# jianwang-mpi/GlobalEgoMocap

Hardware: AMD Instinct MI355X
Metric: optimised windows/sec (10-frame, 15-joint) (higher is better)
Workload: dtype f32

## Files before the change

globalegomocap_amd/csrc/decoder_bf16.hip:

```cpp
#include "gem_internal.h"
#include "gemm_glds.h"
#include "gemm_big.h"

namespace gem {

using glds::Args;
namespace bf16a = glds;

__global__ void f32_to_bf16_kernel(const float* __restrict__ src, uint16_t* __restrict__ dst, size_t n4) {
    const size_t i = (size_t)blockIdx.x * blockDim.x + threadIdx.x;
    if (i >= n4) return;
    const bf16a::f32x4 v = reinterpret_cast<const bf16a::f32x4*>(src)[i];
    reinterpret_cast<bf16a::u32x2*>(dst)[i] = bf16a::u32x2{bf16a::pack_bf16(v[0], v[1]), bf16a::pack_bf16(v[2], v[3])};
}
int launch_f32_to_bf16(const float* src, uint16_t* dst, size_t n, hipStream_t s) {
    const size_t n4 = n / 4;
    if (!n4) return 0;
    hipLaunchKernelGGL(f32_to_bf16_kernel, dim3((unsigned)((n4 + 255) / 256)), dim3(256), 0, s, src, dst, n4);
    GEM_HIP(hipGetLastError());
    return 0;
}

__global__ void f32_split_bf16_kernel(const float* __restrict__ src, uint16_t* __restrict__ hi, uint16_t* __restrict__ lo, size_t n) {
    const size_t i = (size_t)blockIdx.x * blockDim.x + threadIdx.x;
// ... 251 lines not shown
                               nullptr, true, false)) return 1;
                in = w.dec_act_b[i];
            }
        }
        TailArgs ta;
        plan_tail(net.dec, st, T, h->J, &ta);
        ta.B = B; ta.forward_only = forward_only ? 1 : 0; ta.dbg_ts = nullptr;
        ta.in_slab = in_slab; ta.in_bias = front ? net.front.bias : net.dec[st - 1].bias;
        ta.in_bias_ld = front ? net.dec[0].N : 0;
        for (int i = 0; i < ta.n; ++i) {
            const Layer& f = net.dec[st + i];
            const Layer& g = net.dec_bwd[st + i];
            ta.fwd[i] = TailLayerDev{f.w4, f.bias, f.K, f.N};
            ta.bwd[i] = TailLayerDev{g.w4, nullptr, g.K, g.N};
        }
        ta.a_in = w.dec_act[st - 1]; ta.g_out = nullptr; ta.g_out_b = w.dec_grad_b[st];
        ta.Xp = (w.dyn && !forward_only) ? nullptr : w.dec_act.back();
        ta.e = ea;
        if (launch_tail(h, ta, net.tail_lds, s)) return 1;
        if (forward_only) return 0;
        back_from = st - 1;
        gin = w.dec_grad_b[st];
    } else {
        if (front) {
            if (gemm_bf16a(h, net.front, EPI_BIAS_LRELU, w.trial_b, h->Dp, nullptr, w.dec_act_b[0], true, net.front.N, B, s, 0, perm, true, false))
                return 1;
            in = w.dec_act_b[0];
        }
        for (int i = front ? 1 : 0; i < n_dec; ++i) {
            const bool last = i + 1 == n_dec;
// ... 30 lines not shown
```

globalegomocap_amd/csrc/gem_api.hip:

```cpp
#include <cxxabi.h>

#include <algorithm>
#include <cmath>
#include <cstdio>
#include <cstdlib>
#include <cstring>
#include <memory>

#include "gem_internal.h"

namespace gem {

static thread_local std::string g_error;
void set_error(const std::string& msg) { g_error = msg; }
bool hip_ok(hipError_t e, const char* what) {
    if (e == hipSuccess) return true;
    g_error = std::string(what) + ": " + hipGetErrorString(e);
    return false;
}

const char* dev_env(const char* name) {
    const char* on = getenv("GEM_DEV");
    if (!on || on[0] != '1') return nullptr;
    return getenv(name);
// ... 398 lines not shown
        net.dec_bwd.push_back(Lb);
        return 0;
    };
    for (int i = nh - 1; i >= 1; --i)
        if (add_dec(c.hidden[i], c.hidden[i - 1], true, true)) return 1;
    if (add_dec(c.hidden[0], c.hidden[0], true, true)) return 1;
    if (add_dec(c.hidden[0], C, false, false)) return 1;
    net.tail_start = -1;
    if (!dev_env("GEM_NO_TAIL"))
        for (int st = 1; st < (int)net.dec.size(); ++st) {
            const size_t bytes = plan_tail(net.dec, st, T, h->J, nullptr);
            if (bytes && bytes <= 160 * 1024) { net.tail_start = st; net.tail_lds = bytes; break; }
        }
    if (net.tail_start == 1 && !dev_env("GEM_NO_FRONT") && compose_front(h, net, first_conv, dec_in_bias_tm.data())) return 1;
    if (build_tail_bf16_stream(h, net)) return 1;
    net.host_fwd.clear(); net.host_fwd.shrink_to_fit();
    net.host_bwd.clear(); net.host_bwd.shrink_to_fit();
    net.loaded = true;
    return 0;
}

}

namespace gem {

static int check_call(gem_handle* h, int stage, int B, const char* who) {
    if (!h) { set_error(std::string(who) + ": null handle"); return 1; }
    if (stage < 0 || stage > 1 || !h->net[stage].loaded) { set_error(std::string(who) + ": VAE weights of this stage are not loaded"); return 1; }
    if (B < 0 || B > h->ws.Bmax) { set_error(std::string(who) + ": B exceeds max_windows"); return 1; }
    GEM_HIP(hipSetDevice(h->cfg.device));
// ... 109 lines not shown
            if (rc) return 1;
            in = w.dec_act[i];
        }
    }
    TailArgs ta;
    const size_t tail_lds = plan_tail_for(h, net.dec, st, tail_wgs, &ta);
    ta.B = B; ta.forward_only = forward_only ? 1 : 0; ta.dbg_ts = nullptr;
    ta.in_slab = in_slab; ta.in_bias = front ? net.front.bias : net.dec[st - 1].bias;
    ta.in_bias_ld = front ? net.dec[0].N : 0;
    for (int i = 0; i < ta.n; ++i) {
        const Layer& f = net.dec[st + i];
        const Layer& g = net.dec_bwd[st + i];
        ta.fwd[i] = TailLayerDev{f.w4, f.bias, f.K, f.N};
        ta.bwd[i] = TailLayerDev{g.w4, nullptr, g.K, g.N};
    }
    ta.a_in = w.dec_act[st - 1]; ta.g_out = w.dec_grad[st]; ta.g_out_b = nullptr; ta.Xp = (w.dyn && !forward_only) ? nullptr : w.dec_act.back();
    ta.e = ea;
    if (launch_tail(h, ta, tail_lds, s)) return 1;
    if (forward_only) return 0;
    if (front) {
        w.defer_reduce = w.dyn;
        const int rc = launch_gemm(h, net.front_bwd, EPI_BIAS, w.dec_grad[st], net.front_bwd.K, nullptr, w.dz, h->Dp, B, h->T, s, 0);
        w.grad_slab = w.defer_reduce ? w.deferred : SlabSrc{};
        w.defer_reduce = false;
        return rc;
    }
    return decoder_backward(h, stage, B, s, st - 1, w.dec_grad[st]);
}

struct StageRun {
// ... 483 lines not shown
```

globalegomocap_amd/csrc/gem_internal.h:

```cpp
#pragma once
#if defined(__HIP_DEVICE_COMPILE__) && !defined(GEM_NO_PACKED_FP32)
#error "compile with: -Xclang -target-feature -Xclang -packed-fp32-ops -DGEM_NO_PACKED_FP32 (__graft_entry__.NO_PACKED_FP32)"
#endif

#include <hip/hip_runtime.h>
#include <stdint.h>
#include <atomic>
#include <set>
#include <string>
#include <vector>

#include "../../include/gem_hip.h"

namespace gem {

constexpr int PAD = 64;
constexpr float LEAKY_SLOPE = 0.01f;
constexpr double BN_EPS = 1e-5;
constexpr int MAX_HIST = 128;
constexpr int MAXJ_ERR = GEM_MAX_JOINTS;
constexpr int N_LOG = 1 << 16;
constexpr int TRACE_ROUNDS = 64;

inline int pad64(int x) { return (x + PAD - 1) / PAD * PAD; }
// ... 17 lines not shown

struct StageNet {
    bool loaded = false;
    std::vector<Layer> enc;
    Layer fc;
    Layer dec_in;
    std::vector<Layer> dec;
    Layer dec_in_bwd;
    std::vector<Layer> dec_bwd;
    Layer front, front_bwd;
    int tail_start = -1;
    size_t tail_lds = 0;
    uint16_t* tb_stream = nullptr;
    int tb_steps_f = 0, tb_steps_b = 0;
    size_t tb_lds = 0;
    std::vector<std::vector<float>> host_fwd, host_bwd;
    std::vector<void*> allocs;
};

struct alignas(16) LbfgsState {
    int phase, n_iter, evals, ls_iter, ls_evals, max_ls, first_bracket, ls_done, insuf, low, high;
    int hist_count, hist_start, nan_seen;
    double loss, prev_loss, t, gtd, d_norm, H_diag;
    double t_prev, f_prev, gtd_prev;
    double br_t[2], br_f[2], br_gtd[2];
    double ro[MAX_HIST];
    double cadj[MAX_HIST];
};

struct SlabSrc {
// ... 220 lines not shown
struct TailLayerDev { const float* w4; const float* bias; int K, N; };
struct TailArgs {
    int n, B, G, forward_only, escr, mask_first;
    int waves, rows;
    SlabSrc in_slab;
    const float* in_bias;
    int in_bias_ld;
    long long* dbg_ts;
    TailLayerDev fwd[TAIL_MAX_LAYERS], bwd[TAIL_MAX_LAYERS];
    const float* a_in;
    float* g_out;
    uint16_t* g_out_b;
    float* Xp;
    int off_act[TAIL_MAX_LAYERS + 1], ld_act[TAIL_MAX_LAYERS + 1], off_g[2], ld_g, off_red, off_escr, off_zero, off_pre;
    EnergyArgs e;
};
size_t plan_tail(const std::vector<Layer>& dec, int start, int T, int J, TailArgs* out, bool shared = false);
size_t plan_tail_for(const gem_handle* h, const std::vector<Layer>& dec, int start, int wgs, TailArgs* out);

constexpr int TB_MAX_LAYERS = 6;
struct TailB16Layer { int K, N; const float* bias; };
struct TailB16Args {
    int n, B, G, nrt, forward_only, mask_first;
    SlabSrc in_slab;
    const float* in_bias;
    int in_bias_ld;
    const uint16_t* a_in_b;
    uint16_t* g_out_b;
    float* Xp;
    long long* dbg_ts;
    const uint16_t* wstream;
    int steps_f, steps_total;
    TailB16Layer fwd[TB_MAX_LAYERS], bwd[TB_MAX_LAYERS];
    int off_act[TB_MAX_LAYERS + 1], ld_act[TB_MAX_LAYERS + 1];
    int off_mask[TB_MAX_LAYERS], ld_mask[TB_MAX_LAYERS];
    int off_x, escr, off_mb, off_zero, off_tab;
    int off_bwin, off_epair;
    EnergyArgs e;
};
size_t plan_tail_bf16(const std::vector<Layer>& dec, int start, int T, int J, TailB16Args* out, int nrt = 5);
int tail_bf16_row_tiles(const gem_handle* h, int B, int T);
int build_tail_bf16_stream(gem_handle* h, StageNet& net);
int launch_tail_bf16(gem_handle* h, const TailB16Args& a, size_t lds_bytes, hipStream_t s);
int launch_tail(gem_handle* h, const TailArgs& a, size_t lds_bytes, hipStream_t s);
int tail_cap_workgroups(const gem_handle* h, const std::vector<Layer>& dec, int start);
int launch_mean_bone(gem_handle* h, const float* pose, int n_frames, float* out, hipStream_t s);
int launch_gather_windows(const float* frames, const int32_t* frame0, float* out, int B, int T, int JC, hipStream_t s);
int launch_relative_global(const float* local, const double* cams, const int32_t* frame0, float* rel, int B, int T, int J,
                           hipStream_t s);
int launch_to_global(const float* rel, const double* cams, const int32_t* frame0, double* out, int B, int T, int J,
                     hipStream_t s);

int launch_errors(gem_handle* h, const double* est, const double* mid, const double* opt, const double* gt, int F,
                  const double* bone_mm, double* frame_out, double* out, hipStream_t s, int n_seq);
int launch_merge(const double* win, double* tmp, double* out, int n_chunks, int wpc, int T, int JC, int overlap, int smooth,
                 hipStream_t s);
size_t errors_frame_lds_bytes(int J);
// ... 12 lines not shown
```

globalegomocap_amd/csrc/tail.hip:

```cpp
#include <algorithm>

#include "energy_device.h"

namespace gem {

typedef float f32x16 __attribute__((ext_vector_type(16)));
typedef float f32x4 __attribute__((ext_vector_type(4)));

__device__ __forceinline__ float bf16_round(float x) {
    const __bf16 b = (__bf16)x;
    return (float)b;
}

constexpr int TAIL_WAVES = 8;
constexpr int TAIL_THREADS = TAIL_WAVES * 64;
constexpr int TAIL_WAVES_SHARED = 4;

constexpr int TAIL_ROWS = 16;

template <int W>
__device__ __forceinline__ void tail_prefetch_first(const TailLayerDev L, f32x4 (&dst)[4]) {
    const int lane = threadIdx.x & 63, wave = __builtin_amdgcn_readfirstlane(threadIdx.x >> 6);
    const int c = lane & 15, q = lane >> 4;
    const int n0 = wave * 16;
// ... 95 lines not shown
__device__ __forceinline__ void tail_gemm(const float* in, int ld_in, const float* zero_line, const TailLayerDev L,
                                          const TailLayerDev next, bool has_next, int T, int R, f32x4 (&bpre)[4], Epi epi) {
    if constexpr (W == TAIL_WAVES_SHARED) {
        if (L.N > 32 * W) {
            tail_gemm_nt<W, 2>(in, ld_in, zero_line, L, next, false, T, R, bpre, epi);
            tail_gemm_nt<W, 2>(in, ld_in, zero_line, L, next, has_next, T, R, bpre, epi, 32 * W, false);
        } else if (L.N > 16 * W) tail_gemm_nt<W, 2>(in, ld_in, zero_line, L, next, has_next, T, R, bpre, epi);
        else tail_gemm_nt<W, 1>(in, ld_in, zero_line, L, next, has_next, T, R, bpre, epi);
    } else {
        if (L.N > 32 * W) tail_gemm_nt<W, 4>(in, ld_in, zero_line, L, next, has_next, T, R, bpre, epi);
        else if (L.N > 16 * W) tail_gemm_nt<W, 2>(in, ld_in, zero_line, L, next, has_next, T, R, bpre, epi);
        else tail_gemm_nt<W, 1>(in, ld_in, zero_line, L, next, has_next, T, R, bpre, epi);
    }
}

template <int NL, int W>
__global__ __launch_bounds__(64 * W, W == TAIL_WAVES_SHARED ? 3 : 2) void decoder_tail_kernel(TailArgs a) {
    constexpr int THREADS = 64 * W;
    constexpr bool TIGHT = W == TAIL_WAVES_SHARED;
    constexpr int STAGE_U = 2048 / THREADS;
    constexpr int PRE_E = TAIL_THREADS / THREADS;
    extern __shared__ __attribute__((aligned(16))) float lds[];
    const int tid = threadIdx.x, lane = tid & 63, wave = __builtin_amdgcn_readfirstlane(tid >> 6);
    const int T = a.e.T;
    int probe = 0;
#define TAIL_PROBE()                                                                                   \
    if (a.dbg_ts && blockIdx.x == 0 && tid == 0) {                                                     \
        a.dbg_ts[2 * probe] = clock64();                                                               \
        a.dbg_ts[2 * probe + 1] = wall_clock64();                                                      \
        ++probe;                                                                                       \
    }
    const int w0 = blockIdx.x * a.G;
    const int B = a.e.n_dev ? *a.e.n_dev : a.B;
    if (w0 >= B) return;
    const int nwin = min(a.G, B - w0);
    const int R = nwin * T;
    const size_t row0 = (size_t)w0 * T;

    {
        const int K0 = a.fwd[0].K, q4 = K0 / 4, n4 = (TIGHT ? a.rows : TAIL_ROWS) * q4;
        float* dst = lds + a.off_act[0];
        if (a.in_slab.base) {
            int nslab;
            size_t stride;
            slab_layout(a.in_slab, nslab, stride);
            for (int u = 0; u < STAGE_U; ++u) {
                const int i = tid + u * THREADS, r = i / q4, c = (i - r * q4) * 4;
                if (i >= n4) break;
                f32x4 v = {0.f, 0.f, 0.f, 0.f};
                if (r < R) {
                    const float* p = a.in_slab.base + (row0 + r) * K0 + c;
                    for (int z0 = 0; z0 < nslab; z0 += 8) {
                        f32x4 t[8];
#pragma unroll
                        for (int k = 0; k < 8; ++k) t[k] = *reinterpret_cast<const f32x4*>(p + (size_t)min(z0 + k, nslab - 1) * stride);
// ... 10 lines not shown
        } else {
            f32x4 v[STAGE_U];
#pragma unroll
            for (int u = 0; u < STAGE_U; ++u) {
                const int i = tid + u * THREADS, r = i / q4, c = (i - r * q4) * 4;
                v[u] = f32x4{0.f, 0.f, 0.f, 0.f};
                if (i < n4 && r < R) v[u] = *reinterpret_cast<const f32x4*>(a.a_in + (row0 + r) * K0 + c);
            }
#pragma unroll
            for (int u = 0; u < STAGE_U; ++u) {
                const int i = tid + u * THREADS, r = i / q4, c = (i - r * q4) * 4;
                if (i < n4) *reinterpret_cast<f32x4*>(dst + r * a.ld_act[0] + c) = v[u];
            }
        }
        if (tid < 64) lds[a.off_zero + tid] = 0.f;
    }
    float pre_x0[PRE_E], pre_mb = 0.f;
    int pre_par = 0, pre_ch[PRE_E];
#pragma unroll
    for (int k = 0; k < PRE_E; ++k) { pre_x0[k] = 0.f; pre_ch[k] = -1; }
    static_assert(MAXJ * MAXJ <= TAIL_THREADS && MAXJ <= 64, "the children table is parked by PRE_E passes of the workgroup");
    const bool pre_on = a.G == 1 && !a.forward_only && T * a.e.J * 3 <= TAIL_THREADS;
    if (pre_on) {
        const int J = a.e.J, n = T * J * 3, bw = a.e.perm ? a.e.perm[w0] : w0;
#pragma unroll
        for (int k = 0; k < PRE_E; ++k) {
            const int e = tid + k * THREADS;
            if (e < n) pre_x0[k] = a.e.X0[(size_t)bw * n + e];
            if (e < J * MAXJ) pre_ch[k] = a.e.children[e];
        }
        if (tid < J) { pre_mb = a.e.mean_bone[(size_t)bw * J + tid]; pre_par = a.e.parents[tid]; }
    }
    TAIL_PROBE();
    __syncthreads();
    TAIL_PROBE();

    f32x4 bpre[4];
    tail_prefetch_first<W>(a.fwd[0], bpre);
#pragma unroll
    for (int i = 0; i < NL; ++i) {
        const bool last = (i + 1 == NL);
        float* out = lds + a.off_act[i + 1];
        const int ldo = a.ld_act[i + 1];
        float* Xp = last ? a.Xp : nullptr;
        const TailLayerDev nxt = !last ? a.fwd[i + 1 < NL ? i + 1 : i] : a.bwd[NL - 1];
        tail_gemm<W>(lds + a.off_act[i], a.ld_act[i], lds + a.off_zero, a.fwd[i], nxt, !last || !a.forward_only, T, R, bpre,
                  [&](const f32x4& acc, int r0, int col, float bv) {
#pragma unroll
                      for (int e = 0; e < 4; ++e) {
                          float v = acc[e] + bv;
                          if (!last) v = v > 0.f ? v : v * LEAKY_SLOPE;
                          if (!TIGHT || r0 + e < a.rows) out[(r0 + e) * ldo + col] = v;
                          if (Xp && r0 + e < R) Xp[(row0 + r0 + e) * PAD + col] = v;
                      }
                  });
        if (i == 0 && pre_on) {
            const int J = a.e.J, n = T * J * 3;
            float* pre = lds + a.off_pre;
            int* prei = reinterpret_cast<int*>(pre + n + J);
#pragma unroll
            for (int k = 0; k < PRE_E; ++k) {
                const int e = tid + k * THREADS;
                if (e < n) pre[e] = pre_x0[k];
                if (e < J * MAXJ) prei[J + e] = pre_ch[k];
            }
            if (tid < J) { pre[n + tid] = pre_mb; prei[tid] = pre_par; }
        }
        __syncthreads();
        TAIL_PROBE();
    }
    if (a.forward_only) return;

    float* g_cur = lds + a.off_g[0];
    float* g_nxt = lds + a.off_g[1];
    if (a.G == 1) {
        float* scr = lds + a.off_escr;
        const int J = a.e.J, n = T * J * 3;
        const float* pre = lds + a.off_pre;
        const int* prei = reinterpret_cast<const int*>(pre + n + J);
        if (T == 10 && J == 15)
            energy_window<true, THREADS, 10, 15>(a.e, a.e.perm ? a.e.perm[w0] : w0, tid, lds + a.off_act[NL], a.ld_act[NL], scr,
                                                      scr + a.escr, scr + 2 * a.escr, scr + 3 * a.escr, g_cur, a.ld_g, a.fwd[NL - 1].N,
                                                      nullptr, pre_on ? pre : nullptr, pre_on ? pre + n : nullptr, pre_on ? prei : nullptr,
                                                      pre_on ? prei + J : nullptr);
        else
            energy_window<true, THREADS>(a.e, a.e.perm ? a.e.perm[w0] : w0, tid, lds + a.off_act[NL], a.ld_act[NL], scr,
                                              scr + a.escr, scr + 2 * a.escr, scr + 3 * a.escr, g_cur, a.ld_g, a.fwd[NL - 1].N,
                                              nullptr, pre_on ? pre : nullptr, pre_on ? pre + n : nullptr, pre_on ? prei : nullptr,
                                              pre_on ? prei + J : nullptr);
    } else if (wave < nwin) {
        float* scr = lds + a.off_escr + wave * 4 * a.escr;
        energy_window<false>(a.e, a.e.perm ? a.e.perm[w0 + wave] : w0 + wave, lane,
                             lds + a.off_act[NL] + wave * T * a.ld_act[NL], a.ld_act[NL], scr, scr + a.escr,
                             scr + 2 * a.escr, scr + 3 * a.escr, g_cur + wave * T * a.ld_g, a.ld_g, a.fwd[NL - 1].N);
    }
    __syncthreads();
    TAIL_PROBE();

#pragma unroll
    for (int i = NL - 1; i >= 0; --i) {
        const float* act = lds + a.off_act[i];
        const int lda = a.ld_act[i];
        const int ldg = a.ld_g;
        float* gout = a.g_out;
        uint16_t* gout_b = a.g_out_b;
        const int K0 = a.fwd[0].K;
        tail_gemm<W>(g_cur, a.ld_g, lds + a.off_zero, a.bwd[i], a.bwd[i > 0 ? i - 1 : 0], i > 0, T, R, bpre,
                  [&](const f32x4& acc, int r0, int col, float) {
#pragma unroll
                      for (int e = 0; e < 4; ++e) {
                          const int row = r0 + e;
                          const float v = (i > 0 || a.mask_first) ? acc[e] * (act[row * lda + col] > 0.f ? 1.f : LEAKY_SLOPE) : acc[e];
                          if (i > 0) { if (!TIGHT || row < a.rows) g_nxt[row * ldg + col] = v; }
                          else if (row < R) {
                              if (gout_b) gout_b[(row0 + row) * K0 + col] = (uint16_t)(__builtin_bit_cast(unsigned int, bf16_round(v)) >> 16);
                              else gout[(row0 + row) * K0 + col] = v;
                          }
                      }
                  });
        __syncthreads();
        TAIL_PROBE();
        float* t = g_cur; g_cur = g_nxt; g_nxt = t;
    }
#undef TAIL_PROBE
}

size_t plan_tail(const std::vector<Layer>& dec, int start, int T, int J, TailArgs* out, bool shared) {
    const int n = (int)dec.size() - start;
    if (start < 0 || n < 1 || n > TAIL_MAX_LAYERS || T > TAIL_ROWS) return 0;
    for (int i = start; i < (int)dec.size(); ++i) {
        const int K = dec[i].K, N = dec[i].N;
        auto ok = [](int v) { return v == 64 || v == 128 || v == 256 || v == 512; };
        if (!ok(K) || !ok(N)) return 0;
    }
    TailArgs a{};
    a.n = n;
    a.mask_first = start > 0;
    a.G = TAIL_ROWS / T;
    if (shared && a.G != 1) return 0;
// ... 7 lines not shown
        a.ld_act[i] = width + 4;
        off += rows * (width + 4);
        if (i >= 1 && width > maxg) maxg = width;
    }
    a.ld_g = maxg + 4;
    a.off_g[0] = off; off += rows * a.ld_g;
    a.off_g[1] = off; off += rows * a.ld_g;
    a.escr = (T * J * 3 + 3) / 4 * 4;
    a.off_red = off;
    a.off_escr = off;
    off += a.G * 4 * a.escr;
    a.off_zero = off;
    off += 64;
    a.off_pre = off;
    if (a.G == 1) off += (T * J * 3 + 2 * J + J * MAXJ + 3) / 4 * 4;
    if (out) *out = a;
    return (size_t)off * sizeof(float);
}

template <int NL, int W>
static void launch_tail_as(gem_handle* h, const TailArgs& a, int wgs, size_t lds_bytes, hipStream_t s) {
    note_kernel(h, reinterpret_cast<const void*>(decoder_tail_kernel<NL, W>));
    hipLaunchKernelGGL((decoder_tail_kernel<NL, W>), dim3(wgs), dim3(64 * W), lds_bytes, s, a);
}

template <int W>
static int launch_tail_w(gem_handle* h, const TailArgs& a, int wgs, size_t lds_bytes, hipStream_t s) {
    switch (a.n) {
        case 1: launch_tail_as<1, W>(h, a, wgs, lds_bytes, s); break;
        case 2: launch_tail_as<2, W>(h, a, wgs, lds_bytes, s); break;
        case 3: launch_tail_as<3, W>(h, a, wgs, lds_bytes, s); break;
        case 4: launch_tail_as<4, W>(h, a, wgs, lds_bytes, s); break;
        case 5: launch_tail_as<5, W>(h, a, wgs, lds_bytes, s); break;
        case 6: launch_tail_as<6, W>(h, a, wgs, lds_bytes, s); break;
        default: set_error("launch_tail: unsupported number of fused layers"); return 1;
    }
// ... 7 lines not shown
        if (dec[i].N > 64 * TAIL_WAVES_SHARED || dec[i].K > 64 * TAIL_WAVES_SHARED) return false;
    return true;
}

size_t plan_tail_for(const gem_handle* h, const std::vector<Layer>& dec, int start, int wgs, TailArgs* out) {
    bool shared = wgs > h->n_cu && tail_can_share_cu(dec, start, h->T, h->J);
    if (const char* f = dev_env("GEM_TAIL_WAVES")) shared = atoi(f) == TAIL_WAVES_SHARED && tail_can_share_cu(dec, start, h->T, h->J);
    return plan_tail(dec, start, h->T, h->J, out, shared);
}

int tail_cap_workgroups(const gem_handle* h, const std::vector<Layer>& dec, int start) {
    if (const char* f = dev_env("GEM_TAIL_CAP")) return atoi(f) * h->n_cu;
    return (tail_can_share_cu(dec, start, h->T, h->J) ? 10 : 5) * h->n_cu;
}

int launch_tail(gem_handle* h, const TailArgs& a, size_t lds_bytes, hipStream_t s) {
    static PerDeviceOnce attr_once;
    if (attr_once.need(h->cfg.device)) {
        const void* ks[] = {reinterpret_cast<const void*>(decoder_tail_kernel<1, 8>), reinterpret_cast<const void*>(decoder_tail_kernel<2, 8>),
                            reinterpret_cast<const void*>(decoder_tail_kernel<3, 8>), reinterpret_cast<const void*>(decoder_tail_kernel<4, 8>),
                            reinterpret_cast<const void*>(decoder_tail_kernel<5, 8>), reinterpret_cast<const void*>(decoder_tail_kernel<6, 8>),
                            reinterpret_cast<const void*>(decoder_tail_kernel<1, 4>), reinterpret_cast<const void*>(decoder_tail_kernel<2, 4>),
                            reinterpret_cast<const void*>(decoder_tail_kernel<3, 4>), reinterpret_cast<const void*>(decoder_tail_kernel<4, 4>),
                            reinterpret_cast<const void*>(decoder_tail_kernel<5, 4>), reinterpret_cast<const void*>(decoder_tail_kernel<6, 4>)};
        for (const void* k : ks) GEM_HIP(hipFuncSetAttribute(k, hipFuncAttributeMaxDynamicSharedMemorySize, 160 * 1024));
    }
    Profile::Rec rec;
    const bool prof = h->prof.on;
    if (prof) {
        GEM_HIP(hipEventCreate(&rec.a)); GEM_HIP(hipEventCreate(&rec.b));
        rec.family = 1;
        double per_window = 0.0;
        for (int i = 0; i < a.n; ++i) per_window += 2.0 * 3.0 * a.fwd[i].K * a.fwd[i].N * a.e.T;
        if (!a.forward_only) per_window *= 2.0;
        rec.flops = per_window * a.B;
        if (h->ws.dyn) { rec.log_idx = h->ws.cur_log; rec.flops_per_window = per_window; }
        GEM_HIP(hipEventRecord(rec.a, s));
    }
    const int wgs = (a.B + a.G - 1) / a.G;
    if (a.waves != TAIL_WAVES && a.waves != TAIL_WAVES_SHARED) { set_error("launch_tail: the arguments do not come from plan_tail"); return 1; }
    if (a.waves == TAIL_WAVES_SHARED ? launch_tail_w<TAIL_WAVES_SHARED>(h, a, wgs, lds_bytes, s) : launch_tail_w<TAIL_WAVES>(h, a, wgs, lds_bytes, s))
        return 1;
    GEM_HIP(hipGetLastError());
    if (prof) { GEM_HIP(hipEventRecord(rec.b, s)); h->prof.recs.push_back(rec); }
    commit_kernel_names(h, prof ? 1 : -1);
    return 0;
}

}
```

Before: 32100.

## Stream tail weights through per-wave LDS ring via async global-to-LDS loads

Adds a per-wave LDS ring buffer fed by global_load_lds DMA. It streams prepacked fp32 tail weights (built by a new build_tail_stream) into the fused decoder tail GEMMs, with explicit waitcnt and sched_group_barrier interleaving of the loads and MFMAs. Biases and the energy precompute tables are staged in LDS up front instead of in registers. The aim is to hide weight-fetch latency behind MFMA work across layers. It costs extra LDS for the ring, fixes one window per workgroup, and relies on hand-tuned wait counts that are fragile.

```diff
diff --git a/globalegomocap_amd/csrc/decoder_bf16.hip b/globalegomocap_amd/csrc/decoder_bf16.hip
--- a/globalegomocap_amd/csrc/decoder_bf16.hip
+++ b/globalegomocap_amd/csrc/decoder_bf16.hip
@@ -289,6 +289,7 @@
             ta.fwd[i] = TailLayerDev{f.w4, f.bias, f.K, f.N};
             ta.bwd[i] = TailLayerDev{g.w4, nullptr, g.K, g.N};
         }
+        ta.wstream = net.tail_stream; ta.wstream_stride = net.tail_stream_stride; ta.wstream_n = ta.n;
         ta.a_in = w.dec_act[st - 1]; ta.g_out = nullptr; ta.g_out_b = w.dec_grad_b[st];
         ta.Xp = (w.dyn && !forward_only) ? nullptr : w.dec_act.back();
         ta.e = ea;
diff --git a/globalegomocap_amd/csrc/gem_api.hip b/globalegomocap_amd/csrc/gem_api.hip
--- a/globalegomocap_amd/csrc/gem_api.hip
+++ b/globalegomocap_amd/csrc/gem_api.hip
@@ -436,6 +436,7 @@
         }
     if (net.tail_start == 1 && !dev_env("GEM_NO_FRONT") && compose_front(h, net, first_conv, dec_in_bias_tm.data())) return 1;
     if (build_tail_bf16_stream(h, net)) return 1;
+    if (build_tail_stream(h, net)) return 1;
     net.host_fwd.clear(); net.host_fwd.shrink_to_fit();
     net.host_bwd.clear(); net.host_bwd.shrink_to_fit();
     net.loaded = true;
@@ -575,6 +576,7 @@
         ta.fwd[i] = TailLayerDev{f.w4, f.bias, f.K, f.N};
         ta.bwd[i] = TailLayerDev{g.w4, nullptr, g.K, g.N};
     }
+    ta.wstream = net.tail_stream; ta.wstream_stride = net.tail_stream_stride; ta.wstream_n = ta.n;
     ta.a_in = w.dec_act[st - 1]; ta.g_out = w.dec_grad[st]; ta.g_out_b = nullptr; ta.Xp = (w.dyn && !forward_only) ? nullptr : w.dec_act.back();
     ta.e = ea;
     if (launch_tail(h, ta, tail_lds, s)) return 1;
diff --git a/globalegomocap_amd/csrc/gem_internal.h b/globalegomocap_amd/csrc/gem_internal.h
--- a/globalegomocap_amd/csrc/gem_internal.h
+++ b/globalegomocap_amd/csrc/gem_internal.h
@@ -55,6 +55,8 @@
     uint16_t* tb_stream = nullptr;
     int tb_steps_f = 0, tb_steps_b = 0;
     size_t tb_lds = 0;
+    float* tail_stream = nullptr;
+    int tail_stream_stride = 0;
     std::vector<std::vector<float>> host_fwd, host_bwd;
     std::vector<void*> allocs;
 };
@@ -305,6 +307,9 @@
     float* Xp;
     int off_act[TAIL_MAX_LAYERS + 1], ld_act[TAIL_MAX_LAYERS + 1], off_g[2], ld_g, off_red, off_escr, off_zero, off_pre;
     EnergyArgs e;
+    const float* wstream;
+    int wstream_stride, wstream_n;
+    int off_ring, off_bias[TAIL_MAX_LAYERS];
 };
 size_t plan_tail(const std::vector<Layer>& dec, int start, int T, int J, TailArgs* out, bool shared = false);
 size_t plan_tail_for(const gem_handle* h, const std::vector<Layer>& dec, int start, int wgs, TailArgs* out);
@@ -332,6 +337,7 @@
 size_t plan_tail_bf16(const std::vector<Layer>& dec, int start, int T, int J, TailB16Args* out, int nrt = 5);
 int tail_bf16_row_tiles(const gem_handle* h, int B, int T);
 int build_tail_bf16_stream(gem_handle* h, StageNet& net);
+int build_tail_stream(gem_handle* h, StageNet& net);
 int launch_tail_bf16(gem_handle* h, const TailB16Args& a, size_t lds_bytes, hipStream_t s);
 int launch_tail(gem_handle* h, const TailArgs& a, size_t lds_bytes, hipStream_t s);
 int tail_cap_workgroups(const gem_handle* h, const std::vector<Layer>& dec, int start);
diff --git a/globalegomocap_amd/csrc/tail.hip b/globalegomocap_amd/csrc/tail.hip
--- a/globalegomocap_amd/csrc/tail.hip
+++ b/globalegomocap_amd/csrc/tail.hip
@@ -1,4 +1,5 @@
 #include <algorithm>
+#include <utility>
 
 #include "energy_device.h"
 
@@ -133,12 +134,138 @@
     }
 }
 
-template <int NL, int W>
-__global__ __launch_bounds__(64 * W, W == TAIL_WAVES_SHARED ? 3 : 2) void decoder_tail_kernel(TailArgs a) {
-    constexpr int THREADS = 64 * W;
-    constexpr bool TIGHT = W == TAIL_WAVES_SHARED;
+constexpr int TAIL_RING = 11;
+
+struct TailRing {
+    const unsigned char* src;
+    unsigned char* slots;
+    int total, issued, wr, rd;
+};
+
+__device__ __forceinline__ void tail_ring_issue(TailRing& r) {
+    const int p = min(r.issued, r.total - 1);
+    __builtin_amdgcn_global_load_lds((const __attribute__((address_space(1))) void*)(r.src + (size_t)p * 1024),
+                                     (__attribute__((address_space(3))) void*)(r.slots + r.wr * 1024), 16, 0, 0);
+    ++r.issued;
+    r.wr = r.wr + 1 == TAIL_RING ? 0 : r.wr + 1;
+}
+
+__device__ __forceinline__ void tail_barrier_keep_dma() {
+    asm volatile("s_waitcnt lgkmcnt(0)" ::: "memory");
+    __builtin_amdgcn_s_barrier();
+    asm volatile("" ::: "memory");
+}
+
+template <int NP, typename Epi>
+__device__ __forceinline__ void tail_gemm_ring_np(const float* in, int ld_in, const float* zero_line, const TailLayerDev L,
+                                                  const float* bias_lds, int T, int R, TailRing& ring, bool drained, Epi epi) {
+    constexpr int P = 4;
+    const int tid = threadIdx.x, lane = tid & 63, wave = __builtin_amdgcn_readfirstlane(tid >> 6);
+    const int fr = lane & 15, fq = lane >> 4;
+    const int kb = L.K / 64, nblk = 3 * kb;
+    constexpr int TS = 16 * TAIL_WAVES;
+    const int n0 = wave * 16;
+    if (n0 >= L.N) return;
+    const int row = fr;
+    const int t_row = row % T;
+    const bool row_ok = row < R;
+    const int a_own = row * ld_in + 4 * fq;
+    const int a_zero = (int)(zero_line - in) + 4 * fq;
+    const bool ok_m = row_ok && t_row >= 1, ok_p = row_ok && t_row + 1 < T;
+    const unsigned char* my = ring.slots + lane * 16;
+#define RING_LOAD_B(dst_)                                                                              \
+    {                                                                                                  \
+        _Pragma("unroll") for (int g = 0; g < 4; ++g) {                                                \
+            dst_[g] = *reinterpret_cast<const f32x4*>(my + ring.rd * 1024);                            \
+            ring.rd = ring.rd + 1 == TAIL_RING ? 0 : ring.rd + 1;                                      \
+        }                                                                                              \
+    }
+#define RING_LOAD_A(blk_, dst_)                                                                        \
+    {                                                                                                  \
+        const int tap_ = ((blk_) >= kb) + ((blk_) >= 2 * kb), k0_ = ((blk_) - tap_ * kb) * 64;         \
+        const bool ok_ = tap_ == 0 ? ok_m : (tap_ == 1 ? row_ok : ok_p);                               \
+        const float* arow_ = in + (ok_ ? a_own + (tap_ - 1) * ld_in + k0_ : a_zero);                   \
+        _Pragma("unroll") for (int g = 0; g < 4; ++g) dst_[g] = *reinterpret_cast<const f32x4*>(arow_ + 16 * g); \
+    }
+#define RING_COMPUTE(a_, b_, g0_, g1_)                                                                 \
+    {                                                                                                  \
+        _Pragma("unroll") for (int g = g0_; g < g1_; ++g) {                                            \
+            acc = __builtin_amdgcn_mfma_f32_16x16x4f32(a_[g].x, b_[g].x, acc, 0, 0, 0);               \
+            acc = __builtin_amdgcn_mfma_f32_16x16x4f32(a_[g].y, b_[g].y, acc, 0, 0, 0);               \
+            acc = __builtin_amdgcn_mfma_f32_16x16x4f32(a_[g].z, b_[g].z, acc, 0, 0, 0);               \
+            acc = __builtin_amdgcn_mfma_f32_16x16x4f32(a_[g].w, b_[g].w, acc, 0, 0, 0);               \
+        }                                                                                              \
+    }
+#define RING_STEP(ac_, bc_, an_, bn_, nxt_)                                                            \
+    {                                                                                                  \
+        asm volatile("s_waitcnt lgkmcnt(0)" ::: "memory");                                             \
+        _Pragma("unroll") for (int i_ = 0; i_ < P; ++i_) tail_ring_issue(ring);                        \
+        RING_COMPUTE(ac_, bc_, 0, 2);                                                                  \
+        _Pragma("unroll") for (int i_ = 0; i_ < P; ++i_) { __builtin_amdgcn_sched_group_barrier(0x008, 2, 0); __builtin_amdgcn_sched_group_barrier(0x020, 1, 0); } \
+        __builtin_amdgcn_sched_barrier(0);                                                             \
+        asm volatile("s_waitcnt vmcnt(%0)" ::"n"(TAIL_RING - P) : "memory");                           \
+        RING_LOAD_B(bn_);                                                                              \
+        RING_LOAD_A(nxt_, an_);                                                                        \
+        RING_COMPUTE(ac_, bc_, 2, 4);                                                                  \
+        _Pragma("unroll") for (int i_ = 0; i_ < 4; ++i_) { __builtin_amdgcn_sched_group_barrier(0x008, 1, 0); __builtin_amdgcn_sched_group_barrier(0x100, 2, 0); } \
+        __builtin_amdgcn_sched_barrier(0);                                                             \
+    }
+    f32x4 accs[NP];
+#pragma unroll
+    for (int c = 0; c < NP; ++c) {
+        f32x4 acc = {0.f, 0.f, 0.f, 0.f};
+        f32x4 b0[4], b1[4], a0[4], a1[4];
+        if (c == 0 && drained) asm volatile("s_waitcnt vmcnt(0)" ::: "memory");
+        else asm volatile("s_waitcnt vmcnt(%0)" ::"n"(TAIL_RING - P) : "memory");
+        RING_LOAD_B(b0);
+        RING_LOAD_A(0, a0);
+        const int nsteps = nblk - 1;
+        for (int p = 0; p < nsteps / 2; ++p) {
+            RING_STEP(a0, b0, a1, b1, 2 * p + 1);
+            RING_STEP(a1, b1, a0, b0, 2 * p + 2);
+        }
+        if (nsteps & 1) {
+            RING_STEP(a0, b0, a1, b1, nblk - 1);
+            asm volatile("s_waitcnt lgkmcnt(0)" ::: "memory");
+#pragma unroll
+            for (int i = 0; i < P; ++i) tail_ring_issue(ring);
+            RING_COMPUTE(a1, b1, 0, 4);
+        } else {
+            asm volatile("s_waitcnt lgkmcnt(0)" ::: "memory");
+#pragma unroll
+            for (int i = 0; i < P; ++i) tail_ring_issue(ring);
+            RING_COMPUTE(a0, b0, 0, 4);
+        }
+        accs[c] = acc;
+    }
+#undef RING_STEP
+#undef RING_COMPUTE
+#undef RING_LOAD_A
+#undef RING_LOAD_B
+#pragma unroll
+    for (int c = 0; c < NP; ++c) epi(accs[c], 4 * fq, n0 + TS * c + fr, bias_lds ? bias_lds[n0 + TS * c + fr] : 0.f);
+}
+
+template <typename Epi>
+__device__ __forceinline__ void tail_gemm_ring(const float* in, int ld_in, const float* zero_line, const TailLayerDev L,
+                                               const float* bias_lds, int T, int R, TailRing& ring, bool drained, Epi epi) {
+    if (L.N > 16 * TAIL_WAVES) tail_gemm_ring_np<2>(in, ld_in, zero_line, L, bias_lds, T, R, ring, drained, epi);
+    else tail_gemm_ring_np<1>(in, ld_in, zero_line, L, bias_lds, T, R, ring, drained, epi);
+}
+
+__host__ __device__ inline int tail_stream_pieces(int K, int N, int wave) {
+    return 16 * wave < N ? (3 * K / 64) * (N > 16 * TAIL_WAVES ? N / (16 * TAIL_WAVES) : 1) * 4 : 0;
+}
+
+template <int... I, typename F>
+__device__ __forceinline__ void tail_static_for(std::integer_sequence<int, I...>, F&& f) {
+    (f(std::integral_constant<int, I>{}), ...);
+}
+
+template <int NL>
+__device__ __forceinline__ void decoder_tail_ring_body(const TailArgs& a) {
+    constexpr int THREADS = TAIL_THREADS;
     constexpr int STAGE_U = 2048 / THREADS;
-    constexpr int PRE_E = TAIL_THREADS / THREADS;
     extern __shared__ __attribute__((aligned(16))) float lds[];
     const int tid = threadIdx.x, lane = tid & 63, wave = __builtin_amdgcn_readfirstlane(tid >> 6);
     const int T = a.e.T;
@@ -148,16 +275,32 @@
         a.dbg_ts[2 * probe] = clock64();                                                               \
         a.dbg_ts[2 * probe + 1] = wall_clock64();                                                      \
         ++probe;                                                                                       \
-    }
-    const int w0 = blockIdx.x * a.G;
+    }                                                                                                  \
+    if (a.dbg_ts && blockIdx.x == 0 && wave == 0) asm volatile("s_waitcnt vmcnt(0)" ::: "memory");
+    const int w0 = blockIdx.x;
     const int B = a.e.n_dev ? *a.e.n_dev : a.B;
     if (w0 >= B) return;
-    const int nwin = min(a.G, B - w0);
-    const int R = nwin * T;
+    const int R = T;
     const size_t row0 = (size_t)w0 * T;
 
+    TailRing ring;
+    ring.total = 0;
+#pragma unroll
+    for (int i = 0; i < NL; ++i) {
+        ring.total += tail_stream_pieces(a.fwd[i].K, a.fwd[i].N, wave);
+        if (!a.forward_only) ring.total += tail_stream_pieces(a.bwd[i].K, a.bwd[i].N, wave);
+    }
+    ring.src = reinterpret_cast<const unsigned char*>(a.wstream) + (size_t)wave * a.wstream_stride * 1024 + lane * 16;
+    ring.slots = reinterpret_cast<unsigned char*>(lds + a.off_ring) + wave * (TAIL_RING * 1024);
+    ring.issued = 0; ring.wr = 0; ring.rd = 0;
+    if (ring.total > 0) {
+#pragma unroll
+        for (int i = 0; i < TAIL_RING; ++i) tail_ring_issue(ring);
+    }
+
+    const bool pre_on = !a.forward_only && T * a.e.J * 3 <= TAIL_THREADS;
     {
-        const int K0 = a.fwd[0].K, q4 = K0 / 4, n4 = (TIGHT ? a.rows : TAIL_ROWS) * q4;
+        const int K0 = a.fwd[0].K, q4 = K0 / 4, n4 = TAIL_ROWS * q4;
         float* dst = lds + a.off_act[0];
         if (a.in_slab.base) {
             int nslab;
@@ -198,66 +341,49 @@
             }
         }
         if (tid < 64) lds[a.off_zero + tid] = 0.f;
-    }
-    float pre_x0[PRE_E], pre_mb = 0.f;
-    int pre_par = 0, pre_ch[PRE_E];
-#pragma unroll
-    for (int k = 0; k < PRE_E; ++k) { pre_x0[k] = 0.f; pre_ch[k] = -1; }
-    static_assert(MAXJ * MAXJ <= TAIL_THREADS && MAXJ <= 64, "the children table is parked by PRE_E passes of the workgroup");
-    const bool pre_on = a.G == 1 && !a.forward_only && T * a.e.J * 3 <= TAIL_THREADS;
-    if (pre_on) {
-        const int J = a.e.J, n = T * J * 3, bw = a.e.perm ? a.e.perm[w0] : w0;
-#pragma unroll
-        for (int k = 0; k < PRE_E; ++k) {
-            const int e = tid + k * THREADS;
-            if (e < n) pre_x0[k] = a.e.X0[(size_t)bw * n + e];
-            if (e < J * MAXJ) pre_ch[k] = a.e.children[e];
+#pragma unroll
+        for (int i = 0; i < NL; ++i)
+            if (tid < a.fwd[i].N) lds[a.off_bias[i] + tid] = a.fwd[i].bias ? a.fwd[i].bias[tid] : 0.f;
+        if (pre_on) {
+            const int J = a.e.J, n = T * J * 3, bw = a.e.perm ? a.e.perm[w0] : w0;
+            float* pre = lds + a.off_pre;
+            int* prei = reinterpret_cast<int*>(pre + n + J);
+            if (tid < n) pre[tid] = a.e.X0[(size_t)bw * n + tid];
+            if (tid < J * MAXJ) prei[J + tid] = a.e.children[tid];
+            if (tid < J) { pre[n + tid] = a.e.mean_bone[(size_t)bw * J + tid]; prei[tid] = a.e.parents[tid]; }
         }
-        if (tid < J) { pre_mb = a.e.mean_bone[(size_t)bw * J + tid]; pre_par = a.e.parents[tid]; }
     }
     TAIL_PROBE();
     __syncthreads();
     TAIL_PROBE();
 
-    f32x4 bpre[4];
-    tail_prefetch_first<W>(a.fwd[0], bpre);
-#pragma unroll
-    for (int i = 0; i < NL; ++i) {
-        const bool last = (i + 1 == NL);
+    tail_static_for(std::make_integer_sequence<int, NL>{}, [&](auto ic) {
+        constexpr int i = decltype(ic)::value;
+        constexpr bool last = (i + 1 == NL);
         float* out = lds + a.off_act[i + 1];
         const int ldo = a.ld_act[i + 1];
         float* Xp = last ? a.Xp : nullptr;
-        const TailLayerDev nxt = !last ? a.fwd[i + 1 < NL ? i + 1 : i] : a.bwd[NL - 1];
-        tail_gemm<W>(lds + a.off_act[i], a.ld_act[i], lds + a.off_zero, a.fwd[i], nxt, !last || !a.forward_only, T, R, bpre,
-                  [&](const f32x4& acc, int r0, int col, float bv) {
-#pragma unroll
-                      for (int e = 0; e < 4; ++e) {
-                          float v = acc[e] + bv;
-                          if (!last) v = v > 0.f ? v : v * LEAKY_SLOPE;
-                          if (!TIGHT || r0 + e < a.rows) out[(r0 + e) * ldo + col] = v;
-                          if (Xp && r0 + e < R) Xp[(row0 + r0 + e) * PAD + col] = v;
-                      }
-                  });
-        if (i == 0 && pre_on) {
-            const int J = a.e.J, n = T * J * 3;
-            float* pre = lds + a.off_pre;
-            int* prei = reinterpret_cast<int*>(pre + n + J);
-#pragma unroll
-            for (int k = 0; k < PRE_E; ++k) {
-                const int e = tid + k * THREADS;
-                if (e < n) pre[e] = pre_x0[k];
-                if (e < J * MAXJ) prei[J + e] = pre_ch[k];
-            }
-            if (tid < J) { pre[n + tid] = pre_mb; prei[tid] = pre_par; }
-        }
-        __syncthreads();
+        tail_gemm_ring(lds + a.off_act[i], a.ld_act[i], lds + a.off_zero, a.fwd[i], lds + a.off_bias[i], T, R, ring, i == 0,
+                       [&](const f32x4& acc, int r0, int col, float bv) {
+#pragma unroll
+                           for (int e = 0; e < 4; ++e) {
+                               float v = acc[e] + bv;
+                               if (!last) v = v > 0.f ? v : v * LEAKY_SLOPE;
+                               out[(r0 + e) * ldo + col] = v;
+                               if (Xp && r0 + e < R) Xp[(row0 + r0 + e) * PAD + col] = v;
+                           }
+                       });
+        tail_barrier_keep_dma();
         TAIL_PROBE();
-    }
-    if (a.forward_only) return;
+    });
+    if (a.forward_only) {
+        asm volatile("s_waitcnt vmcnt(0)" ::: "memory");
+        return;
+    }
 
     float* g_cur = lds + a.off_g[0];
     float* g_nxt = lds + a.off_g[1];
-    if (a.G == 1) {
+    {
         float* scr = lds + a.off_escr;
         const int J = a.e.J, n = T * J * 3;
         const float* pre = lds + a.off_pre;
@@ -272,41 +398,48 @@
                                               scr + a.escr, scr + 2 * a.escr, scr + 3 * a.escr, g_cur, a.ld_g, a.fwd[NL - 1].N,
                                               nullptr, pre_on ? pre : nullptr, pre_on ? pre + n : nullptr, pre_on ? prei : nullptr,
                                               pre_on ? prei + J : nullptr);
-    } else if (wave < nwin) {
-        float* scr = lds + a.off_escr + wave * 4 * a.escr;
-        energy_window<false>(a.e, a.e.perm ? a.e.perm[w0 + wave] : w0 + wave, lane,
-                             lds + a.off_act[NL] + wave * T * a.ld_act[NL], a.ld_act[NL], scr, scr + a.escr,
-                             scr + 2 * a.escr, scr + 3 * a.escr, g_cur + wave * T * a.ld_g, a.ld_g, a.fwd[NL - 1].N);
     }
     __syncthreads();
     TAIL_PROBE();
 
-#pragma unroll
-    for (int i = NL - 1; i >= 0; --i) {
+    tail_static_for(std::make_integer_sequence<int, NL>{}, [&](auto ic) {
+        constexpr int i = NL - 1 - decltype(ic)::value;
         const float* act = lds + a.off_act[i];
         const int lda = a.ld_act[i];
         const int ldg = a.ld_g;
         float* gout = a.g_out;
         uint16_t* gout_b = a.g_out_b;
         const int K0 = a.fwd[0].K;
-        tail_gemm<W>(g_cur, a.ld_g, lds + a.off_zero, a.bwd[i], a.bwd[i > 0 ? i - 1 : 0], i > 0, T, R, bpre,
-                  [&](const f32x4& acc, int r0, int col, float) {
-#pragma unroll
-                      for (int e = 0; e < 4; ++e) {
-                          const int row = r0 + e;
-                          const float v = (i > 0 || a.mask_first) ? acc[e] * (act[row * lda + col] > 0.f ? 1.f : LEAKY_SLOPE) : acc[e];
-                          if (i > 0) { if (!TIGHT || row < a.rows) g_nxt[row * ldg + col] = v; }
-                          else if (row < R) {
-                              if (gout_b) gout_b[(row0 + row) * K0 + col] = (uint16_t)(__builtin_bit_cast(unsigned int, bf16_round(v)) >> 16);
-                              else gout[(row0 + row) * K0 + col] = v;
-                          }
-                      }
-                  });
-        __syncthreads();
+        tail_gemm_ring(g_cur, a.ld_g, lds + a.off_zero, a.bwd[i], nullptr, T, R, ring, i == NL - 1,
+                       [&](const f32x4& acc, int r0, int col, float) {
+#pragma unroll
+                           for (int e = 0; e < 4; ++e) {
+                               const int row = r0 + e;
+                               const float v = (i > 0 || a.mask_first) ? acc[e] * (act[row * lda + col] > 0.f ? 1.f : LEAKY_SLOPE) : acc[e];
+                               if (i > 0) g_nxt[row * ldg + col] = v;
+                               else if (row < R) {
+                                   if (gout_b) gout_b[(row0 + row) * K0 + col] = (uint16_t)(__builtin_bit_cast(unsigned int, bf16_round(v)) >> 16);
+                                   else gout[(row0 + row) * K0 + col] = v;
+                               }
+                           }
+                       });
+        tail_barrier_keep_dma();
         TAIL_PROBE();
         float* t = g_cur; g_cur = g_nxt; g_nxt = t;
-    }
+    });
+    asm volatile("s_waitcnt vmcnt(0)" ::: "memory");
 #undef TAIL_PROBE
+}
+
+template <int NL, int W>
+__global__ __launch_bounds__(64 * W, W == TAIL_WAVES_SHARED ? 3 : 2) void decoder_tail_kernel(TailArgs a) {
+    if constexpr (W == TAIL_WAVES) { decoder_tail_ring_body<NL>(a); return; }
+#include "tail_w4_body.h"
+}
+template <int NL>
+__global__ __launch_bounds__(TAIL_THREADS, 2) void decoder_tail_w4_kernel(TailArgs a) {
+    constexpr int W = TAIL_WAVES;
+#include "tail_w4_body.h"
 }
 
 size_t plan_tail(const std::vector<Layer>& dec, int start, int T, int J, TailArgs* out, bool shared) {
@@ -344,12 +477,87 @@
     off += 64;
     a.off_pre = off;
     if (a.G == 1) off += (T * J * 3 + 2 * J + J * MAXJ + 3) / 4 * 4;
+    a.off_ring = -1;
+    if (!shared && a.G == 1) {
+        int o = off;
+        for (int i = 0; i < n; ++i) { a.off_bias[i] = o; o += dec[start + i].N; }
+        if ((size_t)(o + TAIL_WAVES * TAIL_RING * 256) * sizeof(float) <= 160 * 1024) { a.off_ring = o; off = o + TAIL_WAVES * TAIL_RING * 256; }
+    }
     if (out) *out = a;
     return (size_t)off * sizeof(float);
 }
 
+int cut_tail_stream(const std::vector<const float*>& fwd, const std::vector<const float*>& bwd, const std::vector<std::pair<int, int>>& dims,
+                    std::vector<float>* out) {
+    const int n = (int)dims.size();
+    int stride = 0;
+    for (int i = 0; i < n; ++i) {
+        if (dims[i].first > 32 * TAIL_WAVES || dims[i].second > 32 * TAIL_WAVES) return 0;
+        stride += tail_stream_pieces(dims[i].first, dims[i].second, 0) + tail_stream_pieces(dims[i].second, dims[i].first, 0);
+    }
+    out->assign((size_t)TAIL_WAVES * stride * 256, 0.f);
+    for (int w = 0; w < TAIL_WAVES; ++w) {
+        float* dst = out->data() + (size_t)w * stride * 256;
+        auto emit = [&](const float* W4, int K, int N) {
+            if (16 * w >= N) return;
+            const int nt = N > 16 * TAIL_WAVES ? N / (16 * TAIL_WAVES) : 1;
+            for (int i = 0; i < nt; ++i)
+                for (int blk = 0; blk < 3 * K / 64; ++blk)
+                    for (int g = 0; g < 4; ++g)
+                        for (int lane = 0; lane < 64; ++lane, dst += 4) {
+                            const float* src = W4 + ((size_t)(16 * blk + 4 * g + (lane >> 4)) * N + 16 * w + 16 * TAIL_WAVES * i + (lane & 15)) * 4;
+                            for (int e = 0; e < 4; ++e) dst[e] = src[e];
+                        }
+        };
+        for (int i = 0; i < n; ++i) emit(fwd[i], dims[i].first, dims[i].second);
+        for (int i = n - 1; i >= 0; --i) emit(bwd[i], dims[i].second, dims[i].first);
+    }
+    return stride;
+}
+
+int build_tail_stream(gem_handle* h, StageNet& net) {
+    net.tail_stream = nullptr; net.tail_stream_stride = 0;
+    const int st = net.tail_start;
+    if (st < 1) return 0;
+    TailArgs plan;
+    if (!plan_tail(net.dec, st, h->T, h->J, &plan) || plan.off_ring < 0) return 0;
+    const int n = (int)net.dec.size() - st;
+    auto to_w4 = [](const std::vector<float>& w, int N, int K) {
+        std::vector<float> o(w.size());
+        for (int t = 0; t < 3; ++t)
+            for (int nn = 0; nn < N; ++nn)
+                for (int k = 0; k < K; ++k) o[(((size_t)t * (K / 4) + k / 4) * N + nn) * 4 + (k & 3)] = w[((size_t)t * N + nn) * K + k];
+        return o;
+    };
+    std::vector<std::vector<float>> wf(n), wb(n);
+    std::vector<const float*> pf(n), pb(n);
+    std::vector<std::pair<int, int>> dims(n);
+    for (int i = 0; i < n; ++i) {
+        const Layer& f = net.dec[st + i];
+        wf[i] = to_w4(net.host_fwd[st + i], f.N, f.K);
+        wb[i] = to_w4(net.host_bwd[st + i], f.K, f.N);
+        pf[i] = wf[i].data(); pb[i] = wb[i].data();
+        dims[i] = {f.K, f.N};
+    }
+    std::vector<float> stream;
+    const int stride = cut_tail_stream(pf, pb, dims, &stream);
+    if (!stride) return 0;
+    void* p = nullptr;
+    GEM_HIP(hipMalloc(&p, stream.size() * sizeof(float)));
+    net.allocs.push_back(p);
+    GEM_HIP(hipMemcpy(p, stream.data(), stream.size() * sizeof(float), hipMemcpyHostToDevice));
+    net.tail_stream = static_cast<float*>(p);
+    net.tail_stream_stride = stride;
+    return 0;
+}
+
 template <int NL, int W>
 static void launch_tail_as(gem_handle* h, const TailArgs& a, int wgs, size_t lds_bytes, hipStream_t s) {
+    if (W == TAIL_WAVES && !a.wstream) {
+        note_kernel(h, reinterpret_cast<const void*>(decoder_tail_w4_kernel<NL>));
+        hipLaunchKernelGGL((decoder_tail_w4_kernel<NL>), dim3(wgs), dim3(64 * W), lds_bytes, s, a);
+        return;
+    }
     note_kernel(h, reinterpret_cast<const void*>(decoder_tail_kernel<NL, W>));
     hipLaunchKernelGGL((decoder_tail_kernel<NL, W>), dim3(wgs), dim3(64 * W), lds_bytes, s, a);
 }
@@ -387,7 +595,7 @@
     return (tail_can_share_cu(dec, start, h->T, h->J) ? 10 : 5) * h->n_cu;
 }
 
-int launch_tail(gem_handle* h, const TailArgs& a, size_t lds_bytes, hipStream_t s) {
+int launch_tail(gem_handle* h, const TailArgs& a_in, size_t lds_bytes, hipStream_t s) {
     static PerDeviceOnce attr_once;
     if (attr_once.need(h->cfg.device)) {
         const void* ks[] = {reinterpret_cast<const void*>(decoder_tail_kernel<1, 8>), reinterpret_cast<const void*>(decoder_tail_kernel<2, 8>),
@@ -395,7 +603,10 @@
                             reinterpret_cast<const void*>(decoder_tail_kernel<5, 8>), reinterpret_cast<const void*>(decoder_tail_kernel<6, 8>),
                             reinterpret_cast<const void*>(decoder_tail_kernel<1, 4>), reinterpret_cast<const void*>(decoder_tail_kernel<2, 4>),
                             reinterpret_cast<const void*>(decoder_tail_kernel<3, 4>), reinterpret_cast<const void*>(decoder_tail_kernel<4, 4>),
-                            reinterpret_cast<const void*>(decoder_tail_kernel<5, 4>), reinterpret_cast<const void*>(decoder_tail_kernel<6, 4>)};
+                            reinterpret_cast<const void*>(decoder_tail_kernel<5, 4>), reinterpret_cast<const void*>(decoder_tail_kernel<6, 4>),
+                            reinterpret_cast<const void*>(decoder_tail_w4_kernel<1>), reinterpret_cast<const void*>(decoder_tail_w4_kernel<2>),
+                            reinterpret_cast<const void*>(decoder_tail_w4_kernel<3>), reinterpret_cast<const void*>(decoder_tail_w4_kernel<4>),
+                            reinterpret_cast<const void*>(decoder_tail_w4_kernel<5>), reinterpret_cast<const void*>(decoder_tail_w4_kernel<6>)};
         for (const void* k : ks) GEM_HIP(hipFuncSetAttribute(k, hipFuncAttributeMaxDynamicSharedMemorySize, 160 * 1024));
     }
     Profile::Rec rec;
@@ -404,13 +615,16 @@
         GEM_HIP(hipEventCreate(&rec.a)); GEM_HIP(hipEventCreate(&rec.b));
         rec.family = 1;
         double per_window = 0.0;
-        for (int i = 0; i < a.n; ++i) per_window += 2.0 * 3.0 * a.fwd[i].K * a.fwd[i].N * a.e.T;
-        if (!a.forward_only) per_window *= 2.0;
-        rec.flops = per_window * a.B;
+        for (int i = 0; i < a_in.n; ++i) per_window += 2.0 * 3.0 * a_in.fwd[i].K * a_in.fwd[i].N * a_in.e.T;
+        if (!a_in.forward_only) per_window *= 2.0;
+        rec.flops = per_window * a_in.B;
         if (h->ws.dyn) { rec.log_idx = h->ws.cur_log; rec.flops_per_window = per_window; }
         GEM_HIP(hipEventRecord(rec.a, s));
     }
-    const int wgs = (a.B + a.G - 1) / a.G;
+    const int wgs = (a_in.B + a_in.G - 1) / a_in.G;
+    TailArgs a = a_in;
+    if (a.wstream && !(a.waves == TAIL_WAVES && a.G == 1 && a.off_ring >= 0 && (a.forward_only ? a.n <= a.wstream_n : a.n == a.wstream_n)))
+        a.wstream = nullptr;
     if (a.waves != TAIL_WAVES && a.waves != TAIL_WAVES_SHARED) { set_error("launch_tail: the arguments do not come from plan_tail"); return 1; }
     if (a.waves == TAIL_WAVES_SHARED ? launch_tail_w<TAIL_WAVES_SHARED>(h, a, wgs, lds_bytes, s) : launch_tail_w<TAIL_WAVES>(h, a, wgs, lds_bytes, s))
         return 1;
diff --git a/globalegomocap_amd/csrc/tail_w4_body.h b/globalegomocap_amd/csrc/tail_w4_body.h
--- /dev/null
+++ b/globalegomocap_amd/csrc/tail_w4_body.h
@@ -0,0 +1,172 @@
+    constexpr int THREADS = 64 * W;
+    constexpr bool TIGHT = W == TAIL_WAVES_SHARED;
+    constexpr int STAGE_U = 2048 / THREADS;
+    constexpr int PRE_E = TAIL_THREADS / THREADS;
+    extern __shared__ __attribute__((aligned(16))) float lds[];
+    const int tid = threadIdx.x, lane = tid & 63, wave = __builtin_amdgcn_readfirstlane(tid >> 6);
+    const int T = a.e.T;
+    int probe = 0;
+#define TAIL_PROBE()                                                                                   \
+    if (a.dbg_ts && blockIdx.x == 0 && tid == 0) {                                                     \
+        a.dbg_ts[2 * probe] = clock64();                                                               \
+        a.dbg_ts[2 * probe + 1] = wall_clock64();                                                      \
+        ++probe;                                                                                       \
+    }
+    const int w0 = blockIdx.x * a.G;
+    const int B = a.e.n_dev ? *a.e.n_dev : a.B;
+    if (w0 >= B) return;
+    const int nwin = min(a.G, B - w0);
+    const int R = nwin * T;
+    const size_t row0 = (size_t)w0 * T;
+
+    {
+        const int K0 = a.fwd[0].K, q4 = K0 / 4, n4 = (TIGHT ? a.rows : TAIL_ROWS) * q4;
+        float* dst = lds + a.off_act[0];
+        if (a.in_slab.base) {
+            int nslab;
+            size_t stride;
+            slab_layout(a.in_slab, nslab, stride);
+            for (int u = 0; u < STAGE_U; ++u) {
+                const int i = tid + u * THREADS, r = i / q4, c = (i - r * q4) * 4;
+                if (i >= n4) break;
+                f32x4 v = {0.f, 0.f, 0.f, 0.f};
+                if (r < R) {
+                    const float* p = a.in_slab.base + (row0 + r) * K0 + c;
+                    for (int z0 = 0; z0 < nslab; z0 += 8) {
+                        f32x4 t[8];
+#pragma unroll
+                        for (int k = 0; k < 8; ++k) t[k] = *reinterpret_cast<const f32x4*>(p + (size_t)min(z0 + k, nslab - 1) * stride);
+#pragma unroll
+                        for (int k = 0; k < 8; ++k)
+                            if (z0 + k < nslab) v += t[k];
+                    }
+                    v += *reinterpret_cast<const f32x4*>(a.in_bias + (r % T) * a.in_bias_ld + c);
+#pragma unroll
+                    for (int q = 0; q < 4; ++q) v[q] = v[q] > 0.f ? v[q] : v[q] * LEAKY_SLOPE;
+                }
+                *reinterpret_cast<f32x4*>(dst + r * a.ld_act[0] + c) = v;
+            }
+        } else {
+            f32x4 v[STAGE_U];
+#pragma unroll
+            for (int u = 0; u < STAGE_U; ++u) {
+                const int i = tid + u * THREADS, r = i / q4, c = (i - r * q4) * 4;
+                v[u] = f32x4{0.f, 0.f, 0.f, 0.f};
+                if (i < n4 && r < R) v[u] = *reinterpret_cast<const f32x4*>(a.a_in + (row0 + r) * K0 + c);
+            }
+#pragma unroll
+            for (int u = 0; u < STAGE_U; ++u) {
+                const int i = tid + u * THREADS, r = i / q4, c = (i - r * q4) * 4;
+                if (i < n4) *reinterpret_cast<f32x4*>(dst + r * a.ld_act[0] + c) = v[u];
+            }
+        }
+        if (tid < 64) lds[a.off_zero + tid] = 0.f;
+    }
+    float pre_x0[PRE_E], pre_mb = 0.f;
+    int pre_par = 0, pre_ch[PRE_E];
+#pragma unroll
+    for (int k = 0; k < PRE_E; ++k) { pre_x0[k] = 0.f; pre_ch[k] = -1; }
+    static_assert(MAXJ * MAXJ <= TAIL_THREADS && MAXJ <= 64, "the children table is parked by PRE_E passes of the workgroup");
+    const bool pre_on = a.G == 1 && !a.forward_only && T * a.e.J * 3 <= TAIL_THREADS;
+    if (pre_on) {
+        const int J = a.e.J, n = T * J * 3, bw = a.e.perm ? a.e.perm[w0] : w0;
+#pragma unroll
+        for (int k = 0; k < PRE_E; ++k) {
+            const int e = tid + k * THREADS;
+            if (e < n) pre_x0[k] = a.e.X0[(size_t)bw * n + e];
+            if (e < J * MAXJ) pre_ch[k] = a.e.children[e];
+        }
+        if (tid < J) { pre_mb = a.e.mean_bone[(size_t)bw * J + tid]; pre_par = a.e.parents[tid]; }
+    }
+    TAIL_PROBE();
+    __syncthreads();
+    TAIL_PROBE();
+
+    f32x4 bpre[4];
+    tail_prefetch_first<W>(a.fwd[0], bpre);
+#pragma unroll
+    for (int i = 0; i < NL; ++i) {
+        const bool last = (i + 1 == NL);
+        float* out = lds + a.off_act[i + 1];
+        const int ldo = a.ld_act[i + 1];
+        float* Xp = last ? a.Xp : nullptr;
+        const TailLayerDev nxt = !last ? a.fwd[i + 1 < NL ? i + 1 : i] : a.bwd[NL - 1];
+        tail_gemm<W>(lds + a.off_act[i], a.ld_act[i], lds + a.off_zero, a.fwd[i], nxt, !last || !a.forward_only, T, R, bpre,
+                  [&](const f32x4& acc, int r0, int col, float bv) {
+#pragma unroll
+                      for (int e = 0; e < 4; ++e) {
+                          float v = acc[e] + bv;
+                          if (!last) v = v > 0.f ? v : v * LEAKY_SLOPE;
+                          if (!TIGHT || r0 + e < a.rows) out[(r0 + e) * ldo + col] = v;
+                          if (Xp && r0 + e < R) Xp[(row0 + r0 + e) * PAD + col] = v;
+                      }
+                  });
+        if (i == 0 && pre_on) {
+            const int J = a.e.J, n = T * J * 3;
+            float* pre = lds + a.off_pre;
+            int* prei = reinterpret_cast<int*>(pre + n + J);
+#pragma unroll
+            for (int k = 0; k < PRE_E; ++k) {
+                const int e = tid + k * THREADS;
+                if (e < n) pre[e] = pre_x0[k];
+                if (e < J * MAXJ) prei[J + e] = pre_ch[k];
+            }
+            if (tid < J) { pre[n + tid] = pre_mb; prei[tid] = pre_par; }
+        }
+        __syncthreads();
+        TAIL_PROBE();
+    }
+    if (a.forward_only) return;
+
+    float* g_cur = lds + a.off_g[0];
+    float* g_nxt = lds + a.off_g[1];
+    if (a.G == 1) {
+        float* scr = lds + a.off_escr;
+        const int J = a.e.J, n = T * J * 3;
+        const float* pre = lds + a.off_pre;
+        const int* prei = reinterpret_cast<const int*>(pre + n + J);
+        if (T == 10 && J == 15)
+            energy_window<true, THREADS, 10, 15>(a.e, a.e.perm ? a.e.perm[w0] : w0, tid, lds + a.off_act[NL], a.ld_act[NL], scr,
+                                                      scr + a.escr, scr + 2 * a.escr, scr + 3 * a.escr, g_cur, a.ld_g, a.fwd[NL - 1].N,
+                                                      nullptr, pre_on ? pre : nullptr, pre_on ? pre + n : nullptr, pre_on ? prei : nullptr,
+                                                      pre_on ? prei + J : nullptr);
+        else
+            energy_window<true, THREADS>(a.e, a.e.perm ? a.e.perm[w0] : w0, tid, lds + a.off_act[NL], a.ld_act[NL], scr,
+                                              scr + a.escr, scr + 2 * a.escr, scr + 3 * a.escr, g_cur, a.ld_g, a.fwd[NL - 1].N,
+                                              nullptr, pre_on ? pre : nullptr, pre_on ? pre + n : nullptr, pre_on ? prei : nullptr,
+                                              pre_on ? prei + J : nullptr);
+    } else if (wave < nwin) {
+        float* scr = lds + a.off_escr + wave * 4 * a.escr;
+        energy_window<false>(a.e, a.e.perm ? a.e.perm[w0 + wave] : w0 + wave, lane,
+                             lds + a.off_act[NL] + wave * T * a.ld_act[NL], a.ld_act[NL], scr, scr + a.escr,
+                             scr + 2 * a.escr, scr + 3 * a.escr, g_cur + wave * T * a.ld_g, a.ld_g, a.fwd[NL - 1].N);
+    }
+    __syncthreads();
+    TAIL_PROBE();
+
+#pragma unroll
+    for (int i = NL - 1; i >= 0; --i) {
+        const float* act = lds + a.off_act[i];
+        const int lda = a.ld_act[i];
+        const int ldg = a.ld_g;
+        float* gout = a.g_out;
+        uint16_t* gout_b = a.g_out_b;
+        const int K0 = a.fwd[0].K;
+        tail_gemm<W>(g_cur, a.ld_g, lds + a.off_zero, a.bwd[i], a.bwd[i > 0 ? i - 1 : 0], i > 0, T, R, bpre,
+                  [&](const f32x4& acc, int r0, int col, float) {
+#pragma unroll
+                      for (int e = 0; e < 4; ++e) {
+                          const int row = r0 + e;
+                          const float v = (i > 0 || a.mask_first) ? acc[e] * (act[row * lda + col] > 0.f ? 1.f : LEAKY_SLOPE) : acc[e];
+                          if (i > 0) { if (!TIGHT || row < a.rows) g_nxt[row * ldg + col] = v; }
+                          else if (row < R) {
+                              if (gout_b) gout_b[(row0 + row) * K0 + col] = (uint16_t)(__builtin_bit_cast(unsigned int, bf16_round(v)) >> 16);
+                              else gout[(row0 + row) * K0 + col] = v;
+                          }
+                      }
+                  });
+        __syncthreads();
+        TAIL_PROBE();
+        float* t = g_cur; g_cur = g_nxt; g_nxt = t;
+    }
+#undef TAIL_PROBE
```

After: 31730. -1.2%, worse.
